# MatteoMer/zolt

Hardware: AMD Instinct MI355X
Metric: BN254 G1 MSM/sec (higher is better)
Workload: dtype u32; 1 GPU; msm_g1_2^20; points=1048576, points_per_gpu=1048576, streams=3, window_bits=17, windows=15, table_levels=15, table_bytes=1006632960, mode=precomputed table of multiples

## Files before the change

zolt_amd/csrc/msm.hip:

```cpp
#include <string.h>

#include <mutex>
#include <vector>

#include "common.hip.h"
#include "g1.hip.h"
#include "g1_29.hip.h"
#include "g1_29x4.hip.h"
#include "msm_plan.h"

#ifndef ZG_TAIL_PRIO
#define ZG_TAIL_PRIO 3
#endif
#define ZG_HIPRIO() __builtin_amdgcn_s_setprio(ZG_TAIL_PRIO)

struct zg_bases_s {
    size_t n = 0;
    int device = -1;
    zg::MsmPlan plan;
    char *d_table = nullptr;
    uint8_t *d_inf = nullptr;
    uint64_t *d_scal = nullptr;
    struct Lane {
        uint32_t *d_dig = nullptr, *d_sorted = nullptr, *d_hist = nullptr, *d_starts = nullptr;
// ... 748 lines not shown
            uint32_t e2 = e1;
            if (p + 2 < b) e1 = sorted[p + 2];
            row = row29_load(table + 64 * (size_t)(e2 & ZG_ROW_MASK));
            rneg = e2 >> 31;
        }
#endif
        if (__builtin_expect(p == kend, 0)) {
            if (q == 0) xyzz29_store(part + 144 * (size_t)(i + r), acc_inf ? xyzz29_identity() : acc);
            acc_inf = true;
            r++;
#ifdef ZG_ACC_RUNEND_STARTS
            kend = starts[nzend[r] + 1];
#else
            asm volatile("v_mov_b32 %0, %1" : "=v"(kend) : "v"(knext));
            knext = nzend[r + 1];
#endif
        }
        uint32_t exc = 0;
        if (QUAD) {
            if (neg) py = f29_neg2(py);
            xyzz29_madd4(acc, acc_inf, px, py, q);
        } else if (__builtin_expect(acc_inf, 0)) {
            xyzz29_start(acc, px, neg ? f29_neg2(py) : py);
            acc_inf = false;
        } else {
#ifdef ZG_ACC_SIGN_BRANCH
            if (neg) py = f29_neg2(py);
            exc = xyzz29_madd_nz(acc, px, py, 0u);
        }
        if (__builtin_expect(exc != 0, 0)) xyzz29_madd_except(acc, acc_inf, px, py, 0u, exc);
#else
            exc = xyzz29_madd_nz(acc, px, py, neg);
        }
        if (__builtin_expect(exc != 0, 0)) xyzz29_madd_except(acc, acc_inf, px, py, neg, exc);
#endif
#ifdef ZG_ACC_ROW_COPY
        row = nxt;
        rneg = nneg;
#endif
    }
    if (q == 0) xyzz29_store(part + 144 * (size_t)(i + r), acc_inf ? xyzz29_identity() : acc);
}

__global__ void __launch_bounds__(64) msm_bucket_combine_kernel(const char *part, const uint32_t *starts, const uint32_t *nzrank, uint32_t NK,
                                                                uint32_t NT, int GS, char *buckets, uint32_t *heavy_list, MsmState *st) {
    ZG_HIPRIO();
    uint32_t t = (blockIdx.x * 64 + threadIdx.x) >> 2, q = threadIdx.x & 3;
    uint32_t k = t / (uint32_t)GS, g = t % (uint32_t)GS;
    XYZZ29 acc = xyzz29_identity();
    bool light = false;
    if (k < NK) {
        uint32_t C = chunk_len(starts[NK], NT);
        uint32_t s0 = starts[k], s1 = starts[k + 1];
        if (s1 == s0) {
            light = true;
        } else {
            uint32_t q0 = s0 / C, q1 = (s1 - 1) / C, cnt = q1 - q0 + 1, base = q0 + nzrank[k];
            if (cnt > 8u * (uint32_t)GS) {
                if (g == 0 && q == 0) {
                    if (cnt > HUGE_PARTIALS) heavy_list[NK + atomicAdd(&st->nhuge, 1u)] = k;
                    else heavy_list[atomicAdd(&st->nheavy, 1u)] = k;
                }
            } else {
                light = true;
                if (g < cnt) acc = xyzz29_load(part + 144 * (size_t)(base + g));
                uint32_t j = g + (uint32_t)GS;
                XYZZ29 nxt = j < cnt ? xyzz29_load(part + 144 * (size_t)(base + j)) : xyzz29_identity();
                while (j < cnt) {
                    XYZZ29 cur = nxt;
                    j += (uint32_t)GS;
                    if (j < cnt) nxt = xyzz29_load(part + 144 * (size_t)(base + j));
                    acc = xyzz29_add4(acc, cur, q);
                }
            }
        }
    }
    for (int d = 1; d < GS; d <<= 1) {
        XYZZ29 o = xyzz29_shfl_down(acc, 4 * d);
        if ((g & (uint32_t)(2 * d - 1)) == 0) acc = xyzz29_add4(acc, o, q);
    }
    if (light && g == 0 && q == 0) xyzz29_store(buckets + 144 * (size_t)k, acc);
}

__device__ __forceinline__ XYZZ29 block_sum_xyzz29(const XYZZ29 &acc, uint4 *sh) {
    uint32_t tid = threadIdx.x;
    xyzz29_store(&sh[tid * 9], acc);
    __syncthreads();
    if (tid < 128) {
        XYZZ29 x = xyzz29_load(&sh[tid * 9]), y = xyzz29_load(&sh[(tid + 128) * 9]);
        xyzz29_store(&sh[tid * 9], xyzz29_add(x, y));
    }
    __syncthreads();
    uint32_t g = tid >> 2, q = tid & 3;
    for (uint32_t o = 64; o > 0; o >>= 1) {
        if (g < o) {
            XYZZ29 x = xyzz29_load(&sh[g * 9]), y = xyzz29_load(&sh[(g + o) * 9]);
            XYZZ29 r = xyzz29_add4(x, y, q);
            if (q == 0) xyzz29_store(&sh[g * 9], r);
        }
        __syncthreads();
    }
    return xyzz29_load(&sh[0]);
}

__device__ __forceinline__ XYZZ29 wave_sum_xyzz29(const XYZZ29 &acc, uint4 *sh) {
    const uint32_t tid = threadIdx.x;
    xyzz29_store(&sh[tid * 9], acc);
    __syncthreads();
    if (tid < 32) {
        XYZZ29 x = xyzz29_load(&sh[tid * 9]), y = xyzz29_load(&sh[(tid + 32) * 9]);
        xyzz29_store(&sh[tid * 9], xyzz29_add(x, y));
    }
    __syncthreads();
    const uint32_t g = tid >> 2, q = tid & 3;
    for (uint32_t o = 16; o > 0; o >>= 1) {
        if (g < o) {
            XYZZ29 x = xyzz29_load(&sh[g * 9]), y = xyzz29_load(&sh[(g + o) * 9]);
            XYZZ29 r = xyzz29_add4(x, y, q);
            if (q == 0) xyzz29_store(&sh[g * 9], r);
        }
        __syncthreads();
    }
    return xyzz29_load(&sh[0]);
}

__global__ void __launch_bounds__(256) msm_heavy_kernel(const char *part, const uint32_t *starts, const uint32_t *nzrank, const uint32_t *nzlist,
                                                        uint32_t NK, uint32_t NT, const uint32_t *heavy_list, MsmState *st, char *part2,
                                                        char *buckets) {
    ZG_HIPRIO();
    __shared__ uint4 sh[256 * 9];
    __shared__ uint32_t sh_last;
    const uint32_t nheavy = st->nheavy, nhuge = st->nhuge;
    if (nheavy == 0 && nhuge == 0) return;
    const uint32_t C = chunk_len(starts[NK], NT), tid = threadIdx.x;
    {
        const uint32_t lane = tid & 63;
        for (uint32_t h = blockIdx.x * 4 + (tid >> 6); h < nheavy; h += gridDim.x * 4) {
            uint32_t k = heavy_list[h];
            uint32_t s0 = starts[k], s1 = starts[k + 1];
            uint32_t q0 = s0 / C, q1 = (s1 - 1) / C, cnt = q1 - q0 + 1, base = q0 + nzrank[k];
            XYZZ29 acc = xyzz29_identity();
            for (uint32_t j = lane; j < cnt; j += 64) acc = xyzz29_add(acc, xyzz29_load(part + 144 * (size_t)(base + j)));
            for (int d = 1; d < 64; d <<= 1) {
                XYZZ29 o = xyzz29_shfl_down(acc, d);
                if ((lane & (uint32_t)(2 * d - 1)) == 0) acc = xyzz29_add(acc, o);
            }
            if (lane == 0) xyzz29_store(buckets + 144 * (size_t)k, acc);
        }
    }
    if (nhuge == 0) return;
    const uint32_t *huge_list = heavy_list + NK;
    uint32_t *arrive = reinterpret_cast<uint32_t *>(st) + 4;
    uint32_t NZ = nzrank[NK];
    uint32_t lo_slot = blockIdx.x * HEAVY_BLOCK_ITEMS, hi_slot = lo_slot + HEAVY_BLOCK_ITEMS;
    if (lo_slot >= NT + NK) return;
    uint32_t lo = 0, hi = NZ;
    while (hi - lo > 1) {
        uint32_t mid = (lo + hi) >> 1;
        if (starts[nzlist[mid]] / C + mid <= lo_slot) lo = mid; else hi = mid;
    }
    for (uint32_t r = lo; r < NZ; r++) {
        uint32_t k = nzlist[r];
        uint32_t s0 = starts[k], s1 = starts[k + 1];
        uint32_t q0 = s0 / C, q1 = (s1 - 1) / C, cnt = q1 - q0 + 1, base = q0 + r;
        if (base >= hi_slot) break;
        if (cnt <= HUGE_PARTIALS || base + cnt <= lo_slot) continue;
        uint32_t r0 = base > lo_slot ? base : lo_slot, r1 = base + cnt < hi_slot ? base + cnt : hi_slot;
        XYZZ29 acc = xyzz29_identity();
        for (uint32_t j = r0 + tid; j < r1; j += 256) acc = xyzz29_add(acc, xyzz29_load(part + 144 * (size_t)j));
        XYZZ29 res = block_sum_xyzz29(acc, sh);
        const uint32_t b0 = base / HEAVY_BLOCK_ITEMS, b1 = (base + cnt - 1) / HEAVY_BLOCK_ITEMS;
        if (tid == 0) {
            xyzz29_store(part2 + 144 * (size_t)(blockIdx.x + r), res);
            uint32_t h = 0;
            while (h < nhuge && huge_list[h] != k) h++;
            uint32_t arrived = __hip_atomic_fetch_add(&arrive[h], 1u, __ATOMIC_ACQ_REL, __HIP_MEMORY_SCOPE_AGENT);
            asm volatile("s_waitcnt vmcnt(0)" ::: "memory");
            sh_last = arrived == b1 - b0 ? 1u : 0u;
        }
        __syncthreads();
        if (sh_last) {
            XYZZ29 a2 = xyzz29_identity();
            for (uint32_t bb = b0 + tid; bb <= b1; bb += 256) a2 = xyzz29_add(a2, xyzz29_load(part2 + 144 * (size_t)(bb + r)));
            __syncthreads();
            XYZZ29 tot = block_sum_xyzz29(a2, sh);
            if (tid == 0) xyzz29_store(buckets + 144 * (size_t)k, tot);
        }
        __syncthreads();
    }
}

__global__ void __launch_bounds__(256) msm_bitsum_kernel(const char *buckets, uint32_t NB, int c, char *out) {
    ZG_HIPRIO();
    __shared__ uint4 sh[256 * 9];
    uint32_t b = blockIdx.y, g = blockIdx.z, PB = gridDim.x;
    uint32_t total = (b == (uint32_t)(c - 1)) ? 1u : NB / 2;
    XYZZ29 acc = xyzz29_identity();
    for (uint32_t j = blockIdx.x * 256 + threadIdx.x; j < total; j += PB * 256) {
        uint32_t k = (b == (uint32_t)(c - 1)) ? NB : ((((j >> b) << 1) | 1u) << b) | (j & ((1u << b) - 1u));
        acc = xyzz29_add(acc, xyzz29_load(buckets + 144 * ((size_t)g * NB + (k - 1))));
    }
    XYZZ29 r = block_sum_xyzz29(acc, sh);
    if (threadIdx.x == 0) xyzz29_store(out + 144 * (((size_t)g * c + b) * PB + blockIdx.x), r);
}

__global__ void __launch_bounds__(256) msm_rowcol_kernel(const char *buckets, uint32_t NB, int lb, int hb, char *rc) {
    ZG_HIPRIO();
    __shared__ uint4 sh[256 * 9];
    const uint32_t x = blockIdx.x, g = blockIdx.y, nrow = 1u << hb, ncol = 1u << lb, t = threadIdx.x;
    XYZZ29 acc = xyzz29_identity();
    const uint32_t len = x < nrow ? ncol : nrow;
    for (uint32_t e = t; e < len; e += 256) {
        const uint32_t k = x < nrow ? ((x << lb) | e) : ((e << lb) | (x - nrow));
        if (k != 0) {
            XYZZ29 v = xyzz29_load(buckets + 144 * ((size_t)g * NB + (k - 1)));
            acc = e < 256 ? v : xyzz29_add(acc, v);
        }
    }
    XYZZ29 r = block_sum_xyzz29(acc, sh);
    if (t == 0) xyzz29_store(rc + 144 * ((size_t)g * (nrow + ncol) + x), r);
}
__global__ void __launch_bounds__(64) msm_rowcol_wave_kernel(const char *buckets, uint32_t NB, int lb, int hb, char *rc) {
    ZG_HIPRIO();
    __shared__ uint4 sh[64 * 9];
    const uint32_t x = blockIdx.x, g = blockIdx.y, nrow = 1u << hb, ncol = 1u << lb, t = threadIdx.x;
    XYZZ29 acc = xyzz29_identity();
    const uint32_t len = x < nrow ? ncol : nrow;
    bool first = true;
    for (uint32_t e = t; e < len; e += 64) {
        const uint32_t k = x < nrow ? ((x << lb) | e) : ((e << lb) | (x - nrow));
        if (k != 0) {
            XYZZ29 v = xyzz29_load(buckets + 144 * ((size_t)g * NB + (k - 1)));
            acc = first ? v : xyzz29_add(acc, v);
            first = false;
        }
    }
    XYZZ29 r = wave_sum_xyzz29(acc, sh);
    if (t == 0) xyzz29_store(rc + 144 * ((size_t)g * (nrow + ncol) + x), r);
}
static void launch_rowcol(hipStream_t st, const char *buckets, uint32_t NB, int lb, int hb, int sets, char *rc) {
    const int wave_from = env_int("ZG_MSM_ROWCOL_WAVE_FROM", 3);
    if (wave_from > 0 && sets >= wave_from)
        hipLaunchKernelGGL(msm_rowcol_wave_kernel, dim3((1u << hb) + (1u << lb), sets), dim3(64), 0, st, buckets, NB, lb, hb, rc);
    else
        hipLaunchKernelGGL(msm_rowcol_kernel, dim3((1u << hb) + (1u << lb), sets), dim3(256), 0, st, buckets, NB, lb, hb, rc);
}

__global__ void __launch_bounds__(256) msm_bits2d_kernel(const char *buckets, const char *rc, uint32_t NB, int c, int lb, int hb, char *out) {
    ZG_HIPRIO();
    __shared__ uint4 sh[256 * 9];
    const uint32_t b = blockIdx.x, g = blockIdx.y, nrow = 1u << hb, ncol = 1u << lb, t = threadIdx.x;
    const char *rcg = rc + 144 * (size_t)g * (nrow + ncol);
    XYZZ29 acc = xyzz29_identity();
    if (b == (uint32_t)(c - 1)) {
        if (t == 0) acc = xyzz29_load(buckets + 144 * ((size_t)g * NB + (NB - 1)));
    } else if (b < (uint32_t)lb) {
        for (uint32_t e = t; e < ncol; e += 256)
            if ((e >> b) & 1u) acc = xyzz29_add(acc, xyzz29_load(rcg + 144 * (size_t)(nrow + e)));
    } else {
        for (uint32_t e = t; e < nrow; e += 256)
            if ((e >> (b - (uint32_t)lb)) & 1u) acc = xyzz29_add(acc, xyzz29_load(rcg + 144 * (size_t)e));
    }
    XYZZ29 r = block_sum_xyzz29(acc, sh);
    if (t == 0) xyzz29_store(out + 144 * ((size_t)g * c + b), r);
}

ZG_DEV void write_result(const XYZZ &acc, int mode, uint64_t *out_rec, uint8_t *out_inf) {
    Affine r;
    bool inf = xyzz_to_affine(acc, r);
    if (mode == 0) {
        affine_store(out_rec, r);
        *out_inf = inf ? 1 : 0;
    } else {
        Fp one = Fp::one();
        if (inf) {
            fe_store(out_rec, one); fe_store(out_rec + 4, one); fe_store(out_rec + 8, Fp::zero());
        } else {
            fe_store(out_rec, r.x); fe_store(out_rec + 4, r.y); fe_store(out_rec + 8, one);
        }
    }
}

ZG_DEV void write_partial_unnormalised(const XYZZ &acc, uint64_t *out_rec) {
    Fp X, Y, Z;
    xyzz_to_jacobian(acc, X, Y, Z);
    fe_store(out_rec, X); fe_store(out_rec + 4, Y); fe_store(out_rec + 8, Z);
}

__global__ void __launch_bounds__(512) msm_final_kernel(const char *bits, int c, int PB, int G, char *rg, int mode, uint64_t *out_rec,
                                                        uint8_t *out_inf, uint32_t rec_stride, uint32_t inf_stride) {
    ZG_HIPRIO();
    __shared__ uint4 pts[256 * 9];
    uint32_t tid = threadIdx.x, g = blockIdx.x, quad = tid >> 2, q = tid & 3;
    uint32_t S = 1;
    while (S < (uint32_t)PB) S <<= 1;
    if (tid < 256) {
        uint32_t b = tid / S, j = tid % S;
        XYZZ29 v = xyzz29_identity();
        if (b < (uint32_t)c && j < (uint32_t)PB) v = xyzz29_load(bits + 144 * (((size_t)g * c + b) * PB + j));
        xyzz29_store(&pts[tid * 9], v);
    }
    __syncthreads();
    for (uint32_t d = 1; d < S; d <<= 1) {
        uint32_t per_bit = S / (2 * d);
        if (quad < (256 / S) * per_bit) {
            uint32_t b = quad / per_bit, j = (quad % per_bit) * 2 * d;
            XYZZ29 x = xyzz29_load(&pts[(b * S + j) * 9]), y = xyzz29_load(&pts[(b * S + j + d) * 9]);
            XYZZ29 r = xyzz29_add4(x, y, q);
            if (q == 0) xyzz29_store(&pts[(b * S + j) * 9], r);
        }
        __syncthreads();
    }
    if (quad < (uint32_t)c) {
        XYZZ29 v = xyzz29_load(&pts[(quad * S) * 9]);
#if !(defined(ZG_EXP_SKIP) && (ZG_EXP_SKIP & 1))
        for (uint32_t i = 0; i < quad; i++) v = xyzz29_dbl4(v, q);
#endif
        if (q == 0) xyzz29_store(&pts[(quad * S) * 9], v);
    }
    __syncthreads();
    uint32_t top = 1;
    while (top < (uint32_t)c) top <<= 1;
    for (uint32_t o = top >> 1; o > 0; o >>= 1) {
        if (quad < o) {
            XYZZ29 x = xyzz29_load(&pts[(quad * S) * 9]), y = xyzz29_load(&pts[((quad + o) * S) * 9]);
            XYZZ29 r = xyzz29_add4(x, y, q);
            if (q == 0) xyzz29_store(&pts[(quad * S) * 9], r);
        }
// ... 515 lines not shown
            uint32_t *d_fbase = ln.d_fine + (size_t)items * ((size_t)1 << q.fb);
            hipLaunchKernelGGL(msm_fine_count_kernel, dim3(items), dim3(1024), 0, st, ln.d_tmp, ln.d_cstarts, d_tst, d_ist, q.NCB, q.fb, q.rb,
                               ln.d_fine);
            hipLaunchKernelGGL(msm_fine_offsets_kernel, dim3(q.NCB), dim3(128), 0, st, d_ist, q.fb, p.NK, ln.d_fine, d_fbase, ln.d_hist);
            hipLaunchKernelGGL(msm_fine_place_kernel, dim3(items), dim3(1024), (STAGE_ENTRIES + 128 + 132) * 4, st, ln.d_tmp, ln.d_cstarts, d_tst,
                               d_ist, q.NCB, q.fb, q.rb, ln.d_fine, d_fbase, sv.sorted, local_shift, (uint32_t)b->n, (uint32_t)off);
        }
        uint32_t tiles = div_up(p.NK, 1024);
        hipLaunchKernelGGL(msm_scan_a_kernel, dim3(tiles), dim3(1024), 0, st, ln.d_hist, p.NK, ln.d_scan_tmp, ln.d_scan_tmp + p.NK,
                           ln.d_scan_tmp + 2 * (size_t)p.NK);
        hipLaunchKernelGGL(msm_scan_b_kernel, dim3(tiles), dim3(1024), 0, st, ln.d_hist, p.NK, ln.d_scan_tmp, ln.d_scan_tmp + p.NK,
                           ln.d_scan_tmp + 2 * (size_t)p.NK, sv.starts, sv.nzrank, sv.nzlist, sv.nzend, reinterpret_cast<uint32_t *>(sv.state),
                           state_words(p.NT, p.NK));
    } else if (q.sort == MsmSort::LDS) {
        uint32_t per_block = (uint32_t)((n + nblk - 1) / nblk);
        prof_begin(ZG_PROF_MSM_DIGITS, st);
        ZG_TRY(launch_digits_lds_c(p.c, st, d_scalars, infp, (uint32_t)n, (uint32_t)n_pts, p.G, per_block, p.NK, nblk, ln.d_dig,
                                   ln.d_blockhist, 0, 0, rows));
        prof_end(ZG_PROF_MSM_DIGITS, st);
        prof_begin(ZG_PROF_MSM_SORT, st);
        hipLaunchKernelGGL(msm_colscan_kernel, dim3(div_up(p.NK, 256)), dim3(256), 0, st, ln.d_blockhist, nblk, p.NK, ln.d_hist);
        {
            uint32_t tiles = div_up(p.NK, 1024);
            hipLaunchKernelGGL(msm_scan_a_kernel, dim3(tiles), dim3(1024), 0, st, ln.d_hist, p.NK, ln.d_scan_tmp, ln.d_scan_tmp + p.NK,
                               ln.d_scan_tmp + 2 * (size_t)p.NK);
            hipLaunchKernelGGL(msm_scan_b_kernel, dim3(tiles), dim3(1024), 0, st, ln.d_hist, p.NK, ln.d_scan_tmp, ln.d_scan_tmp + p.NK,
                               ln.d_scan_tmp + 2 * (size_t)p.NK, sv.starts, sv.nzrank, sv.nzlist, sv.nzend, reinterpret_cast<uint32_t *>(sv.state),
                               state_words(p.NT, p.NK));
        }
        static PerDeviceOnce scatter_once;
        ZG_HIP(scatter_once.run([] {
            return hipFuncSetAttribute(reinterpret_cast<const void *>(msm_scatter_lds_kernel), hipFuncAttributeMaxDynamicSharedMemorySize, 128 * 1024);
        }));
        hipLaunchKernelGGL(msm_scatter_lds_kernel, dim3(nblk), dim3(sort_threads()), p.NK * 4, st, ln.d_dig, (uint32_t)n, (uint32_t)n_pts, p.W, p.G,
                           b->n, (uint32_t)off, per_block, p.NK, sv.starts, ln.d_blockhist, sv.sorted, rowv);
    } else {
        prof_begin(ZG_PROF_MSM_DIGITS, st);
        ZG_HIP(hipMemsetAsync(ln.d_hist, 0, (size_t)p.NK * 4, st));
        ZG_TRY(launch_digits_c(p.c, st, d_scalars, infp, (uint32_t)n, (uint32_t)n_pts, p.G, ln.d_dig, ln.d_hist));
        prof_end(ZG_PROF_MSM_DIGITS, st);
        prof_begin(ZG_PROF_MSM_SORT, st);
        {
            uint32_t tiles = div_up(p.NK, 1024);
            hipLaunchKernelGGL(msm_scan_a_kernel, dim3(tiles), dim3(1024), 0, st, ln.d_hist, p.NK, ln.d_scan_tmp, ln.d_scan_tmp + p.NK,
                               ln.d_scan_tmp + 2 * (size_t)p.NK);
            hipLaunchKernelGGL(msm_scan_b_kernel, dim3(tiles), dim3(1024), 0, st, ln.d_hist, p.NK, ln.d_scan_tmp, ln.d_scan_tmp + p.NK,
                               ln.d_scan_tmp + 2 * (size_t)p.NK, sv.starts, sv.nzrank, sv.nzlist, sv.nzend, reinterpret_cast<uint32_t *>(sv.state),
                               state_words(p.NT, p.NK));
        }
        ZG_HIP(hipMemsetAsync(ln.d_hist, 0, (size_t)p.NK * 4, st));
        hipLaunchKernelGGL(msm_scatter_kernel, dim3(div_up(n, 256), p.W), dim3(256), 0, st, ln.d_dig, (uint32_t)n, (uint32_t)n_pts, p.G,
                           b->n, (uint32_t)off, sv.starts, ln.d_hist, sv.sorted);
    }
    prof_end(ZG_PROF_MSM_SORT, st);
    return ZG_OK;
    };
    auto accumulate_range = [&](size_t n_pts, const SliceView &sv, char *bucket_out) -> int {
    const size_t n = n_pts * (size_t)p.K;
    prof_begin(ZG_PROF_MSM_ACCUMULATE, st);
    bool alone = env_int("ZG_MSM_ALONE_FULL", 1) != 0;
    for (auto &o : b->lanes)
        if (alone && &o != &ln && o.used && o.last_st != st && hipEventQuery(o.done) == hipErrorNotReady) alone = false;
    (void)hipGetLastError();
    if (p.G > 1) alone = true;
    uint32_t NT = chunk_threads((uint64_t)n * p.W, alone);
    if (NT > p.NT || forced_chunk_threads()) NT = p.NT;
    static const unsigned acc_block = [] {
        int v = env_int("ZG_MSM_ACC_BLOCK", 256);
        return (unsigned)(v == 64 || v == 128 ? v : 256);
    }();
#ifdef ZG_ACC_RUNEND_STARTS
    const uint32_t *run_ends = sv.nzlist;
#else
    const uint32_t *run_ends = sv.nzend;
#endif
    if (NT <= (uint32_t)env_int("ZG_MSM_QUAD_ACC_MAX_CHUNKS", 32768))
        hipLaunchKernelGGL(msm_accumulate_chunk_kernel<true>, dim3(div_up((size_t)NT * 4, 256)), dim3(256), 0, st, sv.sorted, sv.starts,
                           sv.nzrank, run_ends, b->d_table, p.NK, NT, ln.d_part);
    else
        hipLaunchKernelGGL(msm_accumulate_chunk_kernel<false>, dim3(div_up(NT, acc_block)), dim3(acc_block), 0, st, sv.sorted, sv.starts,
                           sv.nzrank, run_ends, b->d_table, p.NK, NT, ln.d_part);
    prof_end(ZG_PROF_MSM_ACCUMULATE, st);
    prof_begin(ZG_PROF_MSM_REDUCE, st);
    hipLaunchKernelGGL(msm_bucket_combine_kernel, dim3(div_up((size_t)p.NK * p.GS * 4, 64)), dim3(64), 0, st, ln.d_part, sv.starts,
                       sv.nzrank, p.NK, NT, p.GS, bucket_out, ln.d_heavy, reinterpret_cast<MsmState *>(sv.state));
    uint32_t nblk_a = (NT + p.NK) / HEAVY_BLOCK_ITEMS + 1;
    hipLaunchKernelGGL(msm_heavy_kernel, dim3(nblk_a < 256 ? 256 : nblk_a), dim3(256), 0, st, ln.d_part, sv.starts, sv.nzrank, sv.nzlist,
                       p.NK, NT, ln.d_heavy, reinterpret_cast<MsmState *>(sv.state), ln.d_part2, bucket_out);
    return ZG_OK;
    };
    auto view = [&](size_t j) {
        SliceView sv{ln.d_sorted, ln.d_starts, ln.d_nzrank, ln.d_nzlist, ln.d_nzend, ln.d_state};
        if (S > 1) {
            uint32_t *m = ln.d_slice_meta + j * meta_stride;
            sv = SliceView{ln.d_sorted + j * (size_t)p.W * per, m, m + ((size_t)p.NK + 1), m + 2 * ((size_t)p.NK + 1), m + 3 * ((size_t)p.NK + 1),
                           m + 4 * ((size_t)p.NK + 1)};
        }
        return sv;
    };
    for (size_t j = 0; j < S; j++) {
        const size_t a = j * per, cnt = n_pts - a < per ? n_pts - a : per;
        if (j) prof_end(ZG_PROF_MSM_REDUCE, st);
        ZG_TRY(sort_range(off + a, cnt, d_scalars + 4 * a, view(j)));
        ZG_TRY(accumulate_range(cnt, view(j), j == 0 ? (t_bucket_sink && S == 1 ? t_bucket_sink : ln.d_partial) : ln.d_slice_buckets + (j - 1) * (size_t)p.NK * 144));
    }
    if (t_bucket_sink && S == 1) {
        prof_end(ZG_PROF_MSM_REDUCE, st);
        ZG_HIP(hipGetLastError());
        ZG_HIP(hipEventRecord(ln.done, st));
        return ZG_OK;
    }
    if (S > 1)
        hipLaunchKernelGGL(msm_bucket_fold_kernel, dim3(div_up((size_t)p.NK * 4, 256)), dim3(256), 0, st, ln.d_partial, ln.d_slice_buckets, p.NK,
                           (uint32_t)S);
    if (p.lb) {
        char *d_rc = ln.d_bits + 144 * (size_t)p.G * p.K * p.c;
        launch_rowcol(st, ln.d_partial, p.NB, p.lb, p.hb, p.G * p.K, d_rc);
        hipLaunchKernelGGL(msm_bits2d_kernel, dim3(p.c, p.G * p.K), dim3(256), 0, st, ln.d_partial, d_rc, p.NB, p.c, p.lb, p.hb, ln.d_bits);
    } else {
        hipLaunchKernelGGL(msm_bitsum_kernel, dim3(p.PB, p.c, p.G * p.K), dim3(256), 0, st, ln.d_partial, p.NB, p.c, ln.d_bits);
    }
    hipLaunchKernelGGL(msm_final_kernel, dim3(p.G * p.K), dim3(512), 0, st, ln.d_bits, p.c, p.lb ? 1 : p.PB, p.G, ln.d_rg, mode, d_rec, d_inf_out,
                       rec_stride, inf_stride);
    if (p.G > 1)
        hipLaunchKernelGGL(msm_groups_kernel, dim3(p.K), dim3(4), 0, st, ln.d_rg, p.G, p.c, mode, d_rec, d_inf_out, rec_stride, inf_stride);
    prof_end(ZG_PROF_MSM_REDUCE, st);
    ZG_HIP(hipGetLastError());
    ZG_HIP(hipEventRecord(ln.done, st));
    return ZG_OK;
}

namespace hostfp {
typedef unsigned __int128 u128;
static const uint64_t P[4] = {0x3c208c16d87cfd47ull, 0x97816a916871ca8dull, 0xb85045b68181585dull, 0x30644e72e131a029ull};
static uint64_t n0inv() {
    uint64_t inv = 1;
    for (int i = 0; i < 6; i++) inv *= 2 - P[0] * inv;
    return 0 - inv;
}
static void mul(uint64_t r[4], const uint64_t a[4], const uint64_t b[4]) {
    static const uint64_t N0 = n0inv();
    uint64_t t[6] = {0, 0, 0, 0, 0, 0};
    for (int i = 0; i < 4; i++) {
        u128 c = 0;
        for (int j = 0; j < 4; j++) {
            c += (u128)a[j] * b[i] + t[j];
            t[j] = (uint64_t)c;
            c >>= 64;
        }
        c += t[4];
        t[4] = (uint64_t)c;
        t[5] = (uint64_t)(c >> 64);
        const uint64_t m = t[0] * N0;
        c = ((u128)m * P[0] + t[0]) >> 64;
        for (int j = 1; j < 4; j++) {
            c += (u128)m * P[j] + t[j];
            t[j - 1] = (uint64_t)c;
            c >>= 64;
        }
        c += t[4];
        t[3] = (uint64_t)c;
        t[4] = t[5] + (uint64_t)(c >> 64);
    }
    uint64_t d[4];
    u128 br = 0;
    for (int j = 0; j < 4; j++) {
        u128 v = (u128)t[j] - P[j] - (uint64_t)br;
        d[j] = (uint64_t)v;
        br = (v >> 64) & 1;
    }
    const bool ge = t[4] != 0 || br == 0;
    for (int j = 0; j < 4; j++) r[j] = ge ? d[j] : t[j];
}
static void inv(uint64_t r[4], const uint64_t a[4]) {
    uint64_t e[4] = {P[0] - 2, P[1], P[2], P[3]}, acc[4], base[4];
    bool started = false;
    for (int j = 0; j < 4; j++) base[j] = a[j];
    for (int bit = 253; bit >= 0; bit--) {
        if (started) mul(acc, acc, acc);
        if ((e[bit >> 6] >> (bit & 63)) & 1) {
            if (started) mul(acc, acc, base);
            else {
                for (int j = 0; j < 4; j++) acc[j] = base[j];
                started = true;
            }
        }
    }
    for (int j = 0; j < 4; j++) r[j] = acc[j];
}
static void jacobian_to_affine(const uint64_t rec[12], uint64_t out_xy[8], uint8_t *out_inf) {
    const uint64_t *X = rec, *Y = rec + 4, *Z = rec + 8;
    if ((Z[0] | Z[1] | Z[2] | Z[3]) == 0) {
        for (int i = 0; i < 8; i++) out_xy[i] = 0;
        if (out_inf) *out_inf = 1;
        return;
    }
    uint64_t iz[4], iz2[4], iz3[4];
    inv(iz, Z);
    mul(iz2, iz, iz);
    mul(iz3, iz2, iz);
// ... 480 lines not shown
```

zolt_amd/csrc/msm_plan.h:

```cpp
#pragma once
#include <stdint.h>
#include <stdlib.h>

#include <string>

#include "../../include/zolt_gpu.h"

namespace zg {

void set_error(const std::string &msg);

static constexpr int MAX_GROUPS = 64;
static constexpr uint64_t MAX_BUCKETS = (uint64_t)1 << 21;
static constexpr size_t LDS_SORT_BYTES = 128 * 1024;
static constexpr int ENTRY_BITS = 31;
static constexpr int FINE_BITS_MAX = 7;
static constexpr int FINE_BITS_MIN = 5;
static constexpr uint32_t COARSE_BINS_MAX = 3000;
static constexpr uint32_t TWO_PASS_MIN_BUCKETS = 8192;
static constexpr uint32_t FINE_SLICE = 32768;
static constexpr size_t DEV_SLICES_MAX = 128;
static_assert((uint64_t)COARSE_BINS_MAX << FINE_BITS_MAX <= MAX_BUCKETS && LDS_SORT_BYTES / 4 <= MAX_BUCKETS, "fused sets stay plannable");

enum class MsmSort { ATOMIC, LDS, TWO_PASS };

struct MsmPlan {
    int c;
    int W;
    int L;
    int G;
    uint32_t NB;
    uint32_t NK;
    int K;
    int PB;
    int lb, hb;
    uint32_t NT;
    int GS;
    MsmSort sort;
    int fb;
    int rb;
    uint32_t NCB;
    uint32_t nblk;
};

static inline size_t ceil_div(size_t a, size_t b) { return (a + b - 1) / b; }

static inline int env_int(const char *name, int dflt) {
    const char *v = getenv(name);
    return v && *v ? atoi(v) : dflt;
}

static inline uint32_t forced_chunk_threads() {
    int v = env_int("ZG_MSM_CHUNK_THREADS", 0);
    return v < 1 ? 0u : (uint32_t)v;
}

static inline uint32_t sort_span(uint32_t NK) {
    int v = env_int("ZG_MSM_SORT_SPAN", 0);
    if (v > 0) return (uint32_t)v;
    return NK <= 4096 ? 256u : 2048u;
}

static inline uint32_t two_pass_span(int W) {
    uint32_t cap = W <= 16 ? 2048u : 1024u;
    uint32_t v = (uint32_t)env_int("ZG_MSM_TWO_PASS_SPAN", 2048);
    v = v < 256 ? 256 : v;
    return v > cap ? cap : v;
}

static inline uint32_t chunk_threads(uint64_t digits, bool alone = false) {
    static const uint64_t per_chunk = [] {
        int v = env_int("ZG_MSM_CHUNK_ENTRIES", 16);
        return (uint64_t)(v < 1 ? 1 : v);
    }();
    uint64_t want = digits / per_chunk;
    uint32_t nt = 1024;
    while (nt < want && nt < 131072u) nt <<= 1;
    static const uint32_t inflight = [] {
        int v = env_int("ZG_MSM_INFLIGHT_CHUNKS", 114688);
        return (uint32_t)(v < 1024 ? 1024 : (v > 131072 ? 131072 : v));
    }();
    return nt == 131072u && !alone ? inflight : nt;
}

static int plan_shape(size_t n, const zg_msm_config *cfg, size_t batch, MsmPlan &p) {
    int c = cfg ? cfg->window_bits : 0;
    if (c == 0) c = env_int("ZG_MSM_WINDOW_BITS", 0);
    int L = cfg ? cfg->precompute_levels : 0;
    if (L == 0) L = env_int("ZG_MSM_PRECOMPUTE", 0);
    if (L == 0 && cfg && cfg->expected_uses > 0 && cfg->expected_uses < 16) L = 1;
    if (c == 0 && L == 1) {
        c = n >= ((size_t)1 << 19) ? 15 : (n >= 8192 ? 13 : (n >= 2048 ? 8 : (n >= 64 ? 7 : 5)));
    }
    if (c == 0) {
        c = n >= 32768 ? 16 : (n >= 8192 ? 10 : (n >= 2048 ? 8 : (n >= 64 ? 7 : 5)));
        if (batch == 1 && n >= (size_t)env_int("ZG_MSM_C17_MIN", 900000) && (uint64_t)n * 15 <= ((uint64_t)1 << (ENTRY_BITS - FINE_BITS_MIN))) c = 17;
    }
    if (c < 2 || c > 19) {
        set_error("msm: window_bits must be in [2,19]");
        return ZG_ERR_INVALID;
    }
    p.c = c;
    p.W = (255 + c - 1) / c;
    if (L == 0) L = p.W;
    if (L < 1) L = 1;
    if (L > p.W) L = p.W;
    p.G = (p.W + L - 1) / L;
    p.L = (p.W + p.G - 1) / p.G;
    if (p.G > MAX_GROUPS) {
        set_error("msm: too many bucket groups for this window size");
        return ZG_ERR_INVALID;
    }
    p.NB = 1u << (c - 1);
    p.K = (int)batch;
    if ((uint64_t)p.NB * p.G * batch > MAX_BUCKETS) {
        set_error("msm: too many buckets");
        return ZG_ERR_INVALID;
    }
    p.NK = p.NB * (uint32_t)p.G * (uint32_t)batch;
    const uint32_t forced = forced_chunk_threads();
    p.NT = forced ? forced : chunk_threads((uint64_t)n * batch * p.W, true);
    p.GS = 1;
    const uint64_t nt_usual = forced ? p.NT : chunk_threads((uint64_t)n * batch * p.W);
    while (p.GS < 16 && (uint64_t)p.GS * (uint64_t)env_int("ZG_MSM_COMBINE_PER_QUAD", 4) < nt_usual / p.NK + 1) p.GS <<= 1;
    int pb = (int)(p.NB / 2 / (256 * 4));
    p.PB = pb < 1 ? 1 : (pb > 16 ? 16 : pb);
    if (c > 16 && p.PB > 8) p.PB = 8;
    p.lb = p.hb = 0;
    if (c >= 11 && env_int("ZG_MSM_REDUCE_2D", 1)) {
        p.lb = c / 2;
        p.hb = c - 1 - p.lb;
    }
    return ZG_OK;
}

static inline int fine_bits(size_t table_rows, int fb_max) {
    int need = 1;
    while (((size_t)1 << need) < table_rows) need++;
    return ENTRY_BITS - need < fb_max ? ENTRY_BITS - need : fb_max;
}

static void plan_sort(MsmPlan &p, size_t table_rows, size_t n_total, bool fused) {
    p.fb = p.rb = 0;
    p.NCB = 0;
    if (env_int("ZG_MSM_TWO_PASS_SORT", 1) && p.NK >= TWO_PASS_MIN_BUCKETS && p.W <= 32 && (uint64_t)n_total * p.W >= (1u << 17)) {
        int fb_max = env_int("ZG_MSM_FINE_BITS", FINE_BITS_MAX);
        const int fb = fine_bits(table_rows, fb_max > FINE_BITS_MAX ? FINE_BITS_MAX : fb_max);
        const uint32_t ncb = fb >= env_int("ZG_MSM_FINE_BITS_MIN", FINE_BITS_MIN) ? (p.NK + (1u << fb) - 1) >> fb : 0;
        if (ncb && ncb <= COARSE_BINS_MAX) {
            p.sort = MsmSort::TWO_PASS;
            p.fb = fb;
            p.rb = ENTRY_BITS - fb;
            p.NCB = ncb;
            const uint32_t nblk = (uint32_t)ceil_div(n_total, two_pass_span(p.W));
            p.nblk = nblk < 1 ? 1 : nblk;
            return;
        }
    }
    if ((size_t)p.NK * 4 <= LDS_SORT_BYTES && (fused || env_int("ZG_MSM_LDS_SORT", 1))) {
        p.sort = MsmSort::LDS;
        const uint32_t nblk = (uint32_t)(n_total / (size_t)sort_span(p.NK));
        p.nblk = nblk < 1 ? 1 : (nblk > 256 ? 256 : nblk);
        return;
    }
    p.sort = MsmSort::ATOMIC;
    p.nblk = 0;
}

static int plan_msm(size_t n, const zg_msm_config *cfg, size_t k, size_t table_n, MsmPlan &p, const MsmPlan *within = nullptr) {
    const int rc = plan_shape(n ? n : 1, cfg, k, p);
    if (rc != ZG_OK) return rc;
    if (!within) {
        plan_sort(p, (size_t)p.L * table_n, n * k, k > 1);
        return ZG_OK;
    }
    p.sort = within->sort;
    p.fb = within->fb;
    p.rb = within->rb;
    p.NCB = p.fb ? (p.NK + (1u << p.fb) - 1) >> p.fb : 0;
    p.nblk = within->nblk;
    return ZG_OK;
}

static inline size_t table_span_points(int L) {
    const size_t span_mb = (size_t)env_int("ZG_MSM_TABLE_SPAN_MB", 1024);
    if (!span_mb) return 0;
    const size_t pts = (span_mb << 20) / (64 * (size_t)L), least = (size_t)env_int("ZG_MSM_TABLE_SPAN_MIN_POINTS", 65536);
    return pts < least ? least : pts;
}
static inline void slice_counts(const MsmPlan &p, size_t n_pts, size_t &S, size_t &per) {
    S = 1;
    per = n_pts;
    if (p.K != 1) return;
    const size_t sp = table_span_points(p.L);
    if (!sp || n_pts < 2 * sp) return;
    S = (n_pts + sp - 1) / sp;
    if (S > DEV_SLICES_MAX) S = DEV_SLICES_MAX;
    per = (n_pts + S - 1) / S;
    S = (n_pts + per - 1) / per;
}
static bool slice_sort_plan(const MsmPlan &p, size_t per, MsmPlan &ps, int &shift) {
    shift = 0;
    ps = p;
    if (!env_int("ZG_MSM_SLICE_LOCAL_REFS", 1)) return false;
    int k = 1;
    while (((size_t)1 << k) < per) k++;
    plan_sort(ps, (size_t)p.L << k, per, false);
    if (ps.sort != MsmSort::TWO_PASS || ps.fb <= p.fb) {
        ps = p;
        return false;
    }
    shift = k;
    return true;
}

static inline uint32_t sort_blocks(const MsmPlan &q, size_t n) {
    if (q.sort == MsmSort::TWO_PASS) return (uint32_t)ceil_div(n, two_pass_span(q.W));
    uint32_t nblk = q.nblk;
    while (nblk > 1 && (size_t)(nblk - 1) * 1024 >= n) nblk--;
    return nblk;
}
static inline size_t fine_max_items(const MsmPlan &p, size_t n_total) { return (size_t)p.NCB + (size_t)p.W * n_total / FINE_SLICE + 1; }
struct SortWords {
    size_t blockhist = 0;
    size_t tmp = 0;
    size_t cstarts = 0;
    size_t fine = 0;
    bool fit_in(const SortWords &w) const { return blockhist <= w.blockhist && tmp <= w.tmp && cstarts <= w.cstarts && fine <= w.fine; }
};
static inline SortWords sort_words(const MsmPlan &p, size_t n_total) {
    SortWords w;
    if (p.sort == MsmSort::TWO_PASS) {
        w.blockhist = (size_t)p.nblk * p.NCB;
        w.tmp = (size_t)p.W * n_total + 4 * (size_t)p.NCB + 4;
        w.cstarts = 4 * (size_t)p.NCB + 8;
        w.fine = (fine_max_items(p, n_total) + (size_t)p.NCB) * ((size_t)1 << p.fb);
    } else if (p.sort == MsmSort::LDS) {
        w.blockhist = (size_t)p.nblk * p.NK;
    }
    return w;
}
static inline size_t bitsum_per_group(const MsmPlan &p) {
    const size_t one_d = (size_t)p.c * p.PB, two_d = ((size_t)1 << p.lb) + ((size_t)1 << p.hb) + p.c;
    return p.lb && two_d > one_d ? two_d : one_d;
}

static size_t fuse_set_size(const MsmPlan &hp, size_t table_n, size_t n, size_t k, bool wide_ok, MsmPlan &set) {
    if (n == 0 || k < 2 || !env_int("ZG_MSM_BATCH_FUSE", 1)) return 0;
    const size_t set_buckets = (size_t)hp.NB * hp.G;
    size_t cap = LDS_SORT_BYTES / 4 / set_buckets;
    if (cap < 2 && wide_ok) {
        const int fb = fine_bits((size_t)hp.L * table_n, FINE_BITS_MAX);
        if (fb >= FINE_BITS_MIN) cap = ((size_t)COARSE_BINS_MAX << fb) / set_buckets;
    }
    const size_t by_size = ((size_t)1 << 22) / n;
    if (cap > by_size) cap = by_size;
    if (cap < 2) return 0;
    const size_t kc = k < cap ? k : cap;
    const zg_msm_config cfg{hp.c, hp.L, 0};
    if (plan_msm(n, &cfg, kc, table_n, set) != ZG_OK || set.sort == MsmSort::ATOMIC) return 0;
    return kc;
}

}
```

Baseline: 873.1 MSM/s.

## Add lane-per-bucket combine and LDS tree row/column reduction for MSM tail

Adds a bucket-combine kernel in which each lane walks one bucket's partials serially, replacing the quad-per-group cooperative combine. It also adds a row/column reduction kernel that builds a 4-ary tree in LDS over four lines per workgroup. A planner step picks this LANE tail only for single-set, unsliced plans whose line bits are 6 or 8, with an env override. The aim is to cut shuffle and launch overhead in the reduce tail, at the risk of lane divergence when partial counts are uneven and lower occupancy in the new kernels.

Measured after the change: 884.3 MSM/s, median of 6. +1.3%, better.

```diff
diff --git a/zolt_amd/csrc/msm.hip b/zolt_amd/csrc/msm.hip
--- a/zolt_amd/csrc/msm.hip
+++ b/zolt_amd/csrc/msm.hip
@@ -854,6 +854,42 @@
     if (light && g == 0 && q == 0) xyzz29_store(buckets + 144 * (size_t)k, acc);
 }
 
+__global__ void __launch_bounds__(64) msm_bucket_combine_lane_kernel(const char *part, const uint32_t *starts, const uint32_t *nzrank, uint32_t NK,
+                                                                     uint32_t NT, char *buckets, uint32_t *heavy_list, MsmState *st) {
+    ZG_HIPRIO();
+    const uint32_t k = blockIdx.x * 64 + threadIdx.x;
+    uint32_t cnt = 0, base = 0;
+    bool light = false;
+    if (k < NK) {
+        const uint32_t C = chunk_len(starts[NK], NT);
+        const uint32_t s0 = starts[k], s1 = starts[k + 1];
+        if (s1 == s0) {
+            light = true;
+        } else {
+            const uint32_t q0 = s0 / C, q1 = (s1 - 1) / C, c = q1 - q0 + 1;
+            if (c > 8u) {
+                if (c > HUGE_PARTIALS) heavy_list[NK + atomicAdd(&st->nhuge, 1u)] = k;
+                else heavy_list[atomicAdd(&st->nheavy, 1u)] = k;
+            } else {
+                light = true;
+                cnt = c;
+                base = q0 + nzrank[k];
+            }
+        }
+    }
+    XYZZ29 acc = cnt ? xyzz29_load(part + 144 * (size_t)base) : xyzz29_identity();
+    XYZZ29 nxt = cnt > 1 ? xyzz29_load(part + 144 * (size_t)(base + 1)) : xyzz29_identity();
+    uint32_t j = 1;
+    while (__any(j < cnt)) {
+        const XYZZ29 cur = nxt;
+        const bool on = j < cnt;
+        j++;
+        if (j < cnt) nxt = xyzz29_load(part + 144 * (size_t)(base + j));
+        if (on) acc = xyzz29_add(acc, cur);
+    }
+    if (light) xyzz29_store(buckets + 144 * (size_t)k, acc);
+}
+
 __device__ __forceinline__ XYZZ29 block_sum_xyzz29(const XYZZ29 &acc, uint4 *sh) {
     uint32_t tid = threadIdx.x;
     xyzz29_store(&sh[tid * 9], acc);
@@ -1016,6 +1052,49 @@
         hipLaunchKernelGGL(msm_rowcol_wave_kernel, dim3((1u << hb) + (1u << lb), sets), dim3(64), 0, st, buckets, NB, lb, hb, rc);
     else
         hipLaunchKernelGGL(msm_rowcol_kernel, dim3((1u << hb) + (1u << lb), sets), dim3(256), 0, st, buckets, NB, lb, hb, rc);
+}
+
+__global__ void __launch_bounds__(256) msm_rowcol_lane_kernel(const char *buckets, uint32_t NB, int lb, int hb, char *rc) {
+    namespace lm = lane_map;
+    ZG_HIPRIO();
+    __shared__ uint4 sh[lm::SLOTS * 9];
+    const uint32_t t = threadIdx.x, line0 = blockIdx.x * lm::LINES, g = blockIdx.y, q = t & 3;
+    const int m = lm::line_bits(lb, hb, line0), S = lm::stages(m);
+    const char *bg = buckets + 144 * (size_t)g * NB;
+    if (t < lm::units(m, 1)) {
+        const uint32_t line = line0 + lm::first_line(m, t), e0 = lm::first_element(m, t);
+        auto element = [&](uint32_t i) {
+            const uint32_t k = lm::element(lb, hb, line, e0 + i);
+            return k != 0 ? xyzz29_load(bg + 144 * (size_t)(k - 1)) : xyzz29_identity();
+        };
+        XYZZ29 acc = element(0), nxt = element(1);
+#pragma unroll 1
+        for (uint32_t i = 2; i <= 4; i++) {
+            const XYZZ29 cur = nxt;
+            if (i < 4) nxt = element(i);
+            acc = xyzz29_add(acc, cur);
+        }
+        xyzz29_store(&sh[lm::out_slot(1, t) * 9], acc);
+    }
+    __syncthreads();
+    for (int s = 2; s <= S; s++) {
+        const bool quad = lm::quad_stage(m, s);
+        const uint32_t u = quad ? t >> 2 : t;
+        if (u < lm::units(m, s)) {
+            XYZZ29 acc = xyzz29_load(&sh[lm::in_slot(s, u, 0) * 9]);
+#pragma unroll 1
+            for (uint32_t i = 1; i < 4; i++) {
+                const XYZZ29 v = xyzz29_load(&sh[lm::in_slot(s, u, i) * 9]);
+                acc = quad ? xyzz29_add4(acc, v, q) : xyzz29_add(acc, v);
+            }
+            if (s == S) {
+                if (q == 0) xyzz29_store(rc + 144 * ((size_t)g * ((1u << hb) + (1u << lb)) + line0 + u), acc);
+            } else if (!quad || q == 0) {
+                xyzz29_store(&sh[lm::out_slot(s, u) * 9], acc);
+            }
+        }
+        __syncthreads();
+    }
 }
 
 __global__ void __launch_bounds__(256) msm_bits2d_kernel(const char *buckets, const char *rc, uint32_t NB, int c, int lb, int hb, char *out) {
@@ -1697,8 +1776,12 @@
                            sv.nzrank, run_ends, b->d_table, p.NK, NT, ln.d_part);
     prof_end(ZG_PROF_MSM_ACCUMULATE, st);
     prof_begin(ZG_PROF_MSM_REDUCE, st);
-    hipLaunchKernelGGL(msm_bucket_combine_kernel, dim3(div_up((size_t)p.NK * p.GS * 4, 64)), dim3(64), 0, st, ln.d_part, sv.starts,
-                       sv.nzrank, p.NK, NT, p.GS, bucket_out, ln.d_heavy, reinterpret_cast<MsmState *>(sv.state));
+    if (p.tail == MsmTail::LANE)
+        hipLaunchKernelGGL(msm_bucket_combine_lane_kernel, dim3(div_up(p.NK, 64)), dim3(64), 0, st, ln.d_part, sv.starts, sv.nzrank, p.NK, NT,
+                           bucket_out, ln.d_heavy, reinterpret_cast<MsmState *>(sv.state));
+    else
+        hipLaunchKernelGGL(msm_bucket_combine_kernel, dim3(div_up((size_t)p.NK * p.GS * 4, 64)), dim3(64), 0, st, ln.d_part, sv.starts,
+                           sv.nzrank, p.NK, NT, p.GS, bucket_out, ln.d_heavy, reinterpret_cast<MsmState *>(sv.state));
     uint32_t nblk_a = (NT + p.NK) / HEAVY_BLOCK_ITEMS + 1;
     hipLaunchKernelGGL(msm_heavy_kernel, dim3(nblk_a < 256 ? 256 : nblk_a), dim3(256), 0, st, ln.d_part, sv.starts, sv.nzrank, sv.nzlist,
                        p.NK, NT, ln.d_heavy, reinterpret_cast<MsmState *>(sv.state), ln.d_part2, bucket_out);
@@ -1730,7 +1813,10 @@
                            (uint32_t)S);
     if (p.lb) {
         char *d_rc = ln.d_bits + 144 * (size_t)p.G * p.K * p.c;
-        launch_rowcol(st, ln.d_partial, p.NB, p.lb, p.hb, p.G * p.K, d_rc);
+        if (p.tail == MsmTail::LANE)
+            hipLaunchKernelGGL(msm_rowcol_lane_kernel, dim3(lane_map::workgroups(p.lb, p.hb), 1), dim3(256), 0, st, ln.d_partial, p.NB, p.lb, p.hb, d_rc);
+        else
+            launch_rowcol(st, ln.d_partial, p.NB, p.lb, p.hb, p.G * p.K, d_rc);
         hipLaunchKernelGGL(msm_bits2d_kernel, dim3(p.c, p.G * p.K), dim3(256), 0, st, ln.d_partial, d_rc, p.NB, p.c, p.lb, p.hb, ln.d_bits);
     } else {
         hipLaunchKernelGGL(msm_bitsum_kernel, dim3(p.PB, p.c, p.G * p.K), dim3(256), 0, st, ln.d_partial, p.NB, p.c, ln.d_bits);
diff --git a/zolt_amd/csrc/msm_lane_map.h b/zolt_amd/csrc/msm_lane_map.h
--- /dev/null
+++ b/zolt_amd/csrc/msm_lane_map.h
@@ -0,0 +1,35 @@
+#pragma once
+#include <stdint.h>
+
+#if defined(__HIP__)
+#define ZG_LANE_MAP_FN __attribute__((host)) __attribute__((device)) constexpr
+#else
+#define ZG_LANE_MAP_FN constexpr
+#endif
+
+namespace zg {
+namespace lane_map {
+
+static constexpr uint32_t LINES = 4;
+static constexpr uint32_t SLOTS = 256;
+
+ZG_LANE_MAP_FN bool line_bits_ok(int m) { return m == 6 || m == 8; }
+
+ZG_LANE_MAP_FN uint32_t workgroups(int lb, int hb) { return ((1u << hb) + (1u << lb)) / LINES; }
+ZG_LANE_MAP_FN int line_bits(int lb, int hb, uint32_t line) { return line < (1u << hb) ? lb : hb; }
+ZG_LANE_MAP_FN uint32_t element(int lb, int hb, uint32_t line, uint32_t e) {
+    return line < (1u << hb) ? ((line << lb) | e) : ((e << lb) | (line - (1u << hb)));
+}
+
+ZG_LANE_MAP_FN int stages(int m) { return m / 2; }
+ZG_LANE_MAP_FN uint32_t units(int m, int s) { return (LINES << m) >> (2 * s); }
+ZG_LANE_MAP_FN bool quad_stage(int m, int s) { return s + 2 > stages(m); }
+
+ZG_LANE_MAP_FN uint32_t first_line(int m, uint32_t u) { return u >> (m - 2); }
+ZG_LANE_MAP_FN uint32_t first_element(int m, uint32_t u) { return (u & ((1u << (m - 2)) - 1u)) * 4u; }
+
+ZG_LANE_MAP_FN uint32_t in_slot(int s, uint32_t u, uint32_t i) { return (4u * u + i) << (2 * (s - 2)); }
+ZG_LANE_MAP_FN uint32_t out_slot(int s, uint32_t u) { return u << (2 * (s - 1)); }
+
+}
+}
diff --git a/zolt_amd/csrc/msm_plan.h b/zolt_amd/csrc/msm_plan.h
--- a/zolt_amd/csrc/msm_plan.h
+++ b/zolt_amd/csrc/msm_plan.h
@@ -1,10 +1,12 @@
 #pragma once
 #include <stdint.h>
 #include <stdlib.h>
+#include <string.h>
 
 #include <string>
 
 #include "../../include/zolt_gpu.h"
+#include "msm_lane_map.h"
 
 namespace zg {
 
@@ -23,6 +25,7 @@
 static_assert((uint64_t)COARSE_BINS_MAX << FINE_BITS_MAX <= MAX_BUCKETS && LDS_SORT_BYTES / 4 <= MAX_BUCKETS, "fused sets stay plannable");
 
 enum class MsmSort { ATOMIC, LDS, TWO_PASS };
+enum class MsmTail { QUAD, LANE };
 
 struct MsmPlan {
     int c;
@@ -37,6 +40,7 @@
     uint32_t NT;
     int GS;
     MsmSort sort;
+    MsmTail tail;
     int fb;
     int rb;
     uint32_t NCB;
@@ -167,9 +171,12 @@
     p.nblk = 0;
 }
 
+static inline void plan_tail(MsmPlan &p, size_t n);
+
 static int plan_msm(size_t n, const zg_msm_config *cfg, size_t k, size_t table_n, MsmPlan &p, const MsmPlan *within = nullptr) {
     const int rc = plan_shape(n ? n : 1, cfg, k, p);
     if (rc != ZG_OK) return rc;
+    plan_tail(p, n);
     if (!within) {
         plan_sort(p, (size_t)p.L * table_n, n * k, k > 1);
         return ZG_OK;
@@ -199,6 +206,27 @@
     per = (n_pts + S - 1) / S;
     S = (n_pts + per - 1) / per;
 }
+static inline int lane_tail_switch() {
+    const char *v = getenv("ZG_MSM_LANE_TAIL");
+    if (!v || !*v || !strcmp(v, "auto")) return -1;
+    return atoi(v) != 0;
+}
+static inline void plan_tail(MsmPlan &p, size_t n) {
+    p.tail = MsmTail::QUAD;
+    const int sw = lane_tail_switch();
+    if (sw == 0 || p.K != 1 || p.G != 1 || !p.lb) return;
+    size_t S, per;
+    slice_counts(p, n, S, per);
+    if (S > 1) return;
+    int lb = p.lb, hb = p.hb;
+    if (sw == 1 && lb == hb && (lb & 1)) lb--, hb++;
+    if (!lane_map::line_bits_ok(lb) || !lane_map::line_bits_ok(hb)) return;
+    if (sw < 0 && p.NT > 2 * (uint64_t)p.NK) return;
+    p.tail = MsmTail::LANE;
+    p.lb = lb;
+    p.hb = hb;
+}
+
 static bool slice_sort_plan(const MsmPlan &p, size_t per, MsmPlan &ps, int &shift) {
     shift = 0;
     ps = p;
```
